# dart-icra/DART-Dual-Arm-Non-Prehensile-Manipulation

Hardware: AMD Instinct MI355X
Metric: MPC solves/sec (horizon N=20, batch=18 objects) at 1/2/4/8 GPUs; max |u−u_ref| (higher is better)
Workload: dtype f64

## Files before the change

dart-dual-arm-non-prehensile-manipulation_amd/csrc/dart_mpc_abi.hip:

```cpp
#include <hip/hip_runtime.h>

#include <cstdio>
#include <cstring>
#include <chrono>
#include <mutex>
#include <initializer_list>
#include <vector>
#include <string>

#include "dart_mpc.h"
#include "pmpc_ipm.h"
#include "pmpc_model.h"
#include "wave.h"
#include "rmpc_ipm.h"
#include "lmpc_ipm.h"
#include "lmpc_policy.h"
#include "lmpc_experience.h"
#include "lmpc_ppo.h"
#include "lmpc_train.h"
#include "arm_qp.h"
#include "loop_step.h"

#include <cmath>

// ... 151 lines not shown
        size_t cap;
        int xcd;
    };
    std::vector<RestoArea> resto;
    unsigned xcd_next = 0;
    char* loop_buf = nullptr;
    char* roll_buf = nullptr;
    size_t roll_cap = 0;
    float* action_buf = nullptr;
};

namespace {

int fail(dart_mpc_handle* h, int code, const char* what, hipError_t e = hipSuccess) {
    if (h) {
        char buf[256];
        if (e != hipSuccess) std::snprintf(buf, sizeof buf, "%s: %s", what, hipGetErrorString(e));
        else std::snprintf(buf, sizeof buf, "%s", what);
        h->err = buf;
    }
    return code;
}

#define HIPCHK(h, call, what)                                          \
    do {                                                               \
        hipError_t e_ = (call);                                        \
        if (e_ != hipSuccess) return fail((h), DART_MPC_EHIP, (what), e_); \
    } while (0)

int check_cfg(const dart_mpc_config* c) {
    if (!c) return 0;
    if (c->variant != DART_MPC_PMPC && c->variant != DART_MPC_RMPC && c->variant != DART_MPC_LMPC) return 0;
    if (c->N < 1 || c->N > 63) return 0;
    if (!(c->Ts > 0.0) || !(c->tol > 0.0) || !(c->gravity == c->gravity) || c->max_iter < 1 || c->B_max < 1) return 0;
    if (c->acceptable_iter < 0 || (c->acceptable_iter > 0 && !(c->acceptable_tol > 0.0))) return 0;
    if (c->max_soc < 0 || c->max_soc > 8) return 0;
    if (c->pmpc_path != 0 && c->pmpc_path != 1) return 0;
    if (!(c->constr_mult_init_max >= 0.0)) return 0;
    if (!(c->max_cpu_time >= 0.0) || c->max_cpu_time > 1e9) return 0;
    return 1;
}

void server_release(dart_mpc_handle* h) {
    auto& v = h->srv;
    if (v.mbox) (void)hipHostFree(v.mbox);
    if (v.stream) (void)hipStreamDestroy(v.stream);
    v = dart_mpc_handle::Server{};
}

void io_release(dart_mpc_handle* h) {
    auto& o = h->io;
    if (o.hin) (void)hipHostFree(o.hin);
    if (o.hout) (void)hipHostFree(o.hout);
    o = dart_mpc_handle::Io{};
}

hipError_t ensure_io(dart_mpc_handle* h) {
    auto& o = h->io;
    if (o.hin) return hipSuccess;
    const size_t nw = (size_t)dart_mpc_nw(h->cfg.N), Bm = (size_t)h->cfg.B_max;
    auto al = [](size_t n) { return (n + 255) & ~size_t(255); };
    o.off_ref = al(sizeof(double) * 6 * Bm); o.off_prm = 2 * o.off_ref; o.off_ww = 3 * o.off_ref;
    const size_t in_bytes = o.off_ww + al(sizeof(double) * nw * Bm);
    o.off_f = al(sizeof(double) * 2 * Bm); o.off_wo = o.off_f + al(sizeof(double) * Bm);
    o.off_st = o.off_wo + al(sizeof(double) * nw * Bm); o.off_it = o.off_st + al(sizeof(int32_t) * Bm);
    const size_t out_bytes = o.off_it + al(sizeof(int32_t) * Bm);
    const unsigned fl = hipHostMallocMapped | hipHostMallocCoherent;
// ... 2565 lines not shown
```

dart-dual-arm-non-prehensile-manipulation_amd/csrc/pmpc_ipm.hip:

```cpp
#if DART_WG == 2
#define dartmpc dartmpc_wg2
#endif
#include <hip/hip_runtime.h>
#include <stdint.h>
#include <stdlib.h>

#include "pmpc_ipm.h"
#include "pmpc_model.h"
#include "pmpc_resto.h"
#include "stamps.h"
#include "wave.h"

namespace dartmpc {

#ifdef DART_STAMPS
#ifndef PMPC_SEQ
__device__ unsigned long long g_stamp[16];
#define STAMP_FLUSH(b) STAMP_FLUSH_TO(g_stamp, b)
#else
__device__ unsigned long long g_stamp_seq[16];
#define STAMP_FLUSH(b) STAMP_FLUSH_TO(g_stamp_seq, b)
#endif
#else
#define STAMP_FLUSH(b) STAMP_FLUSH_TO(g_stamp, b)
#endif

#if DART_WG == 2
__shared__ double g_pm_x[4][2][4];
#endif
template <int SITE, int NV>
__device__ __forceinline__ void pm_pass(int src_wave, int src_node, const double (&v)[NV], double (&o)[NV]) {
    static_assert(NV <= 4 && SITE < 4, "four slots, four sites");
#if DART_WG == 1
    (void)src_wave; (void)src_node;
#pragma unroll
    for (int i = 0; i < NV; ++i) o[i] = v[i];
#else
    const int l = lane_id();
    if (wave_idx() == src_wave && (l & 31) == src_node) {
#pragma unroll
        for (int i = 0; i < NV; ++i) g_pm_x[SITE][l >> 5][i] = v[i];
    }
    __syncthreads();
#pragma unroll
    for (int i = 0; i < NV; ++i) o[i] = g_pm_x[SITE][l >> 5][i];
#endif
}

template <int CTRL, int ROWMASK, int FILL>
__device__ __forceinline__ double dpp_fill(double x) {
    const unsigned long long b = __builtin_bit_cast(unsigned long long, x);
// ... 205 lines not shown
        const double iQ = frcp(Q);
        W1[0] = iQ * U1; W2[0] = iQ * U2;
        Quu[0] = Q; iQs[0] = iQ;
    } else
    for (int step = 0; step < N; ++step) {
        double n11[NAX], n12[NAX], n22[NAX];
#pragma unroll
        for (int j = 0; j < NAX; ++j) {
            n11[j] = from_next(P11[j]); n12[j] = from_next(P12[j]); n22[j] = from_next(P22[j]);
        }
#pragma unroll
        for (int j = 0; j < NAX; ++j) {
            const double e1 = be1[j], e2 = be2[j];
            const double Q = fma(E11[j], n11[j], fma(E12[j], n12[j], fma(E22[j], n22[j], Rt[j])));
            const double PB1 = fma(n11[j], e1, n12[j] * e2), PB2 = fma(n12[j], e1, n22[j] * e2);
            const double U1 = PB1, U2 = fma(PB1, a12k, PB2 * a22k);
            const double X12 = fma(n11[j], a12k, n12[j] * a22k);
            const double X22 = fma(A11k, n11[j], fma(A12k, n12[j], fma(A22k, n22[j], X22d)));
            const double iQ = frcp(Q);
            const double w1 = iQ * U1, w2 = iQ * U2;
            P11[j] = fma(-w1, U1, fma(f11, n11[j], X11d));
            P12[j] = fma(-w1, U2, X12);
            P22[j] = fma(-w2, U2, X22);
            W1[j] = w1; W2[j] = w2;
            Quu[j] = Q; iQs[j] = iQ;
        }
    }
    bool bad = false;
#pragma unroll
    for (int j = 0; j < NAX; ++j) bad = bad || !(Quu[j] > 0.0) || !isfinite(Quu[j]);
    return !wany(bad);
}

struct PmOvlShared {
    double pt[6][kWave];
    double fc[6][kWave];
    int flag[4];
};
__shared__ PmOvlShared g_pm_ovl;

template <int NAX, bool QSCAN, bool ONEROW, bool SHORT2, bool RED, bool OVL = false>
__device__ __forceinline__ bool pmpc_solve(const PmpcArgs& a, const int b) {
    static_assert(!OVL || (NAX == 1 && QSCAN && !ONEROW && !RED && kWaves == 1), "the overlapped build: scan builds of N = 16..31");
    STAMP_DECL
    const int lane = (kWaves == 1 && !OVL) ? (int)threadIdx.x : lane_id();
    const int k = NAX == 1 ? node_base() + (lane & 31) : lane;
    const int ax0 = NAX == 1 ? (lane >> 5) : 0;
    const int N = a.N;
    const bool xon = k <= N, uon = k < N;
    constexpr bool one_row = ONEROW;
    constexpr bool short2 = SHORT2 && !ONEROW;
    const double h = a.Ts;

    const double* st = a.x0 + 6 * b;
    const double* rf = a.ref + 6 * b;
    const double* pr = a.prm + 6 * b;
    const double mu_f = pr[0], Qp = pr[1], Qv = pr[2], R = pr[3], ulo = pr[4], uhi = pr[5];

    double a12, a22, b1, b2;
    axis_rk4(h, a.g, mu_f, 0.0, 0.0, 1.0, a12, a22);
    axis_rk4(h, a.g, mu_f, 1.0, 0.0, 0.0, b1, b2);
    double zp1, zav, zcp, zcv;
    z_rk4(h, 0.0, 1.0, 1.0, zp1, zav);
    z_rk4(h, 1.0, 0.0, 0.0, zcp, zcv);
    const double lo = ulo - 1e-8 * fmax(1.0, fabs(ulo));
    const double hi = uhi + 1e-8 * fmax(1.0, fabs(uhi));
    const bool poly = fmax(fabs(lo), fabs(hi)) <= 1.0;
    const double f11 = uon ? 1.0 : 0.0, a12k = uon ? a12 : 0.0, a22k = uon ? a22 : 0.0;
    const double ai22 = 1.0 / a22, ai12 = -a12 * ai22;
    const double uonf = uon ? 1.0 : 0.0, ai12k = uon ? ai12 : 0.0, ai22k = uon ? ai22 : 1.0, a22i = uon ? a22 : 1.0;
    const double A11k = a12k * a12k, A12k = 2.0 * a12k * a22k, A22k = a22k * a22k;

// ... 5 lines not shown
    const double pushl = fmin(1e-2 * fmax(1.0, fabs(lo)), 1e-2 * (hi - lo));
    const double pushu = fmin(1e-2 * fmax(1.0, fabs(hi)), 1e-2 * (hi - lo));
    double gmax = 0.0;
#pragma unroll
    for (int j = 0; j < NAX; ++j) {
        const int ax = NAX == 1 ? ax0 : j;
        sp[j] = st[2 * ax]; sv[j] = st[2 * ax + 1];
        rp[j] = rf[2 * ax]; rv[j] = rf[2 * ax + 1];
        p[j] = xon ? (ww ? ww[6 * k + 2 * ax] : sp[j]) : 0.0;
        v[j] = xon ? (ww ? ww[6 * k + 2 * ax + 1] : sv[j]) : 0.0;
        double t = uon ? (ww ? ww[6 * (N + 1) + 2 * k + ax] : 0.0) : 0.0;
        if (uon) t = fmin(fmax(t, lo + pushl), hi - pushu);
        th[j] = t;
        lp[j] = 0.0; lv[j] = 0.0;
        zl[j] = uon ? 1.0 : 0.0; zu[j] = uon ? 1.0 : 0.0;
        if (xon) gmax = fmax(gmax, fmax(fabs(2 * Qp * (p[j] - rp[j])), fabs(2 * Qv * (v[j] - rv[j]))));
        if (uon) gmax = fmax(gmax, fabs(2 * R * th[j]));
        zA[j] = ax ? zav : zp1; zC[j] = ax ? zcv : zcp;
        zs[j] = st[4 + ax];
        zz[j] = xon ? (ww ? ww[6 * k + 4 + ax] : zs[j]) : 0.0;
    }
    gmax = wmax(gmax);
    const double sc = gmax > 100.0 ? 100.0 / gmax : 1.0;
    const double qp2 = sc * 2 * Qp, qv2 = sc * 2 * Qv, r2 = sc * 2 * R;
    const double scQp = sc * Qp, scQv = sc * Qv, scR = sc * R;
    const PmStage stg = {f11, a12k, a22k, ai12k, ai22k, a22i, uonf, A11k, A12k, A22k};
    auto quad_stage = [&](double csj, double snj, double lpnj, double lvnj, double zlj, double islj, double zuj,
                          double isuj, double& e1, double& e2, double& e11, double& e12, double& e22, double& rt0) {
        e1 = b1 * csj; e2 = b2 * csj;
        e11 = e1 * e1; e12 = 2.0 * e1 * e2; e22 = e2 * e2;
        rt0 = uon ? fma(snj, fma(b1, lpnj, b2 * lvnj), r2 + zlj * islj + zuj * isuj) : 1.0;
    };
    if constexpr (OVL) {
        if (__builtin_amdgcn_readfirstlane((int)(threadIdx.x >> 6)) != 0) {
            const long long max_rounds = 2ll * a.max_iter + 8;
            for (long long round = 0; round < max_rounds; ++round) {
                __syncthreads();
                if (__builtin_amdgcn_readfirstlane(g_pm_ovl.flag[0])) return false;
#ifdef DART_STAMPS
                const unsigned long long tf0 = __builtin_amdgcn_s_memtime();
#endif
                const double th1 = g_pm_ovl.pt[0][lane], sn1 = g_pm_ovl.pt[1][lane];
                const double lp1 = g_pm_ovl.pt[2][lane], lv1 = g_pm_ovl.pt[3][lane];
                const double zl1 = g_pm_ovl.pt[4][lane], zu1 = g_pm_ovl.pt[5][lane];
                const double c_ = tilt_cos_econ(poly, th1);
                const double cs1 = uon ? c_ : 0.0;
                const double ln = from_next(lp1), vn = from_next(lv1);
                const double lpn1 = uon ? ln : 0.0, lvn1 = uon ? vn : 0.0;
                const double sl = th1 - lo, su = hi - th1;
                const double isl1 = uon ? frcp(sl) : 0.0, isu1 = uon ? frcp(su) : 0.0;
                double be1[NAX], be2[NAX], E11[NAX], E12[NAX], E22[NAX], Rt0[NAX];
                quad_stage(cs1, sn1, lpn1, lvn1, zl1, isl1, zu1, isu1, be1[0], be2[0], E11[0], E12[0], E22[0], Rt0[0]);
                double W1[NAX], W2[NAX], P11[NAX], P12[NAX], P22[NAX], iQs[NAX];
                bool us = false;
                const bool okf = pmpc_riccati<NAX, QSCAN, ONEROW, SHORT2>(lane, N, uon, false, 0.0, qp2, qv2, stg, be1,
                                                                         be2, E11, E12, E22, Rt0, P11, P12, P22, W1,
                                                                         W2, iQs, us);
                g_pm_ovl.fc[0][lane] = P11[0]; g_pm_ovl.fc[1][lane] = P12[0]; g_pm_ovl.fc[2][lane] = P22[0];
                g_pm_ovl.fc[3][lane] = W1[0]; g_pm_ovl.fc[4][lane] = W2[0]; g_pm_ovl.fc[5][lane] = iQs[0];
                if (lane == 0) { g_pm_ovl.flag[1] = us ? 1 : 0; g_pm_ovl.flag[2] = okf ? 1 : 0; }
#ifdef DART_STAMPS
                t_acc_[13] += __builtin_amdgcn_s_memtime() - tf0;
                if (lane == 0) g_pm_ovl.flag[3] = (int)t_acc_[13];
#endif
                __syncthreads();
                if (__builtin_amdgcn_readfirstlane(g_pm_ovl.flag[0])) return false;
            }
            return false;
        }
        if (lane == 0) g_pm_ovl.flag[0] = 0;
    }

    const double tol = a.tol, mu_min = tol / 10;
    const double n_eq = 6.0 * (N + 1), n_b = 4.0 * N;
    const double inv_neb = 1.0 / (n_eq + n_b), inv_nb = 1.0 / n_b;
    const double gam_th = 1e-5, gam_ph = 1e-8, s_th = 1.1, s_ph = 2.3, eta_ph = 1e-8, gam_al = 0.05;

    auto defects = [&](double pj, double vj, double sj, double spj, double svj, double& g1, double& g2) {
        const double fp = fma(a12, vj, fma(b1, sj, pj));
        const double fv = fma(a22, vj, b2 * sj);
        double ip, iv;
        if constexpr (kWaves == 1) {
            ip = from_prev(fp); iv = from_prev(fv);
        } else {
            const double x2[2] = {fp, fv};
            double o2[2];
            from_prev_n(x2, o2);
            ip = o2[0]; iv = o2[1];
        }
        g1 = (k == 0) ? pj - spj : pj - ip;
        g2 = (k == 0) ? vj - svj : vj - iv;
    };
    auto axes_sum = [&](const double (&q)[NAX]) -> double {
        if constexpr (NAX == 1) return half_pair_sum(q[0]);
        else return q[0] + q[1];
    };
    auto zdefect = [&](double zj, double wj, int j) -> double {
        const double fz = fma(zA[j], zj, zC[j] * wj);
        const double ip = from_prev(fz);
        return (k == 0) ? zj - zs[j] : zj - ip;
    };
    auto vz_new = [&](const double (&t)[NAX]) -> double {
        double sq[NAX];
#pragma unroll
        for (int j = 0; j < NAX; ++j) sq[j] = uon ? t[j] * t[j] : 0.0;
        return -a.g * axes_sum(sq);
    };

    double g1[NAX], g2[NAX], gz[NAX], snc[NAX];
    double th0 = 0.0;
    {
        const double w0 = vz_new(th);
#pragma unroll
        for (int j = 0; j < NAX; ++j) {
            double s0, c0_;
            tilt_sincos(poly, th[j], s0, c0_);
            snc[j] = uon ? s0 : 0.0;
            defects(p[j], v[j], snc[j], sp[j], sv[j], g1[j], g2[j]);
            gz[j] = RED ? 0.0 : zdefect(zz[j], w0, j);
            if (xon) th0 += fabs(g1[j]) + fabs(g2[j]) + fabs(gz[j]);
        }
    }
    double theta = wsum(th0);
    const double th_max = 1e4 * fmax(1.0, theta), th_min = 1e-4 * fmax(1.0, theta);

    double fth = 0.0, fph = 0.0;
    int nfilt = 0;
    double mu = 0.1, delta_last = 0.0;
    int status = -1, it = 0;
    int in_soft = 0, soft_count = 0;
    STAMP(0);

    bool published = false;
    auto publish = [&]() {
        __builtin_amdgcn_sched_barrier(0);
        g_pm_ovl.pt[0][lane] = th[0]; g_pm_ovl.pt[1][lane] = snc[0];
        g_pm_ovl.pt[2][lane] = lp[0]; g_pm_ovl.pt[3][lane] = lv[0];
        g_pm_ovl.pt[4][lane] = zl[0]; g_pm_ovl.pt[5][lane] = zu[0];
        __syncthreads();
        __builtin_amdgcn_sched_barrier(0);
        published = true;
    };
#ifdef DART_STAMPS
    const unsigned long long t_loop0 = __builtin_amdgcn_s_memtime();
#endif
    for (it = a.mult_init_max > 0.0 ? -1 : 0; it < a.max_iter; ++it) {
        const bool lsm = it < 0;
#ifdef DART_STAMPS
        if (it == 1) t_acc_[12] = __builtin_amdgcn_s_memtime() - t_loop0;
#endif
        if constexpr (OVL) {
            if (PM_EXPECT(!lsm && !published, 0)) publish();
        }
        double sn[NAX], cs[NAX], isl[NAX], isu[NAX], lpn[NAX], lvn[NAX];
        double dinf = 0.0, pinf = 0.0, c0 = 0.0, cmin = 1e300, suml = 0.0, sumz = 0.0;
#pragma unroll
        for (int j = 0; j < NAX; ++j) {
            sn[j] = snc[j];
            const double c_ = tilt_cos_econ(poly, th[j]);
            cs[j] = uon ? c_ : 0.0;
            double ln, vn;
            if constexpr (kWaves == 1) {
                ln = from_next(lp[j]); vn = from_next(lv[j]);
            } else {
                const double x2[2] = {lp[j], lv[j]};
                double o2[2];
                from_next_n(x2, o2);
                ln = o2[0]; vn = o2[1];
            }
            lpn[j] = uon ? ln : 0.0; lvn[j] = uon ? vn : 0.0;
            const double sl = th[j] - lo, su = hi - th[j];
            isl[j] = uon ? frcp(sl) : 0.0; isu[j] = uon ? frcp(su) : 0.0;
            const double r1 = fma(qp2, p[j] - rp[j], lp[j] - lpn[j]);
            const double r2x = fma(qv2, v[j] - rv[j], lv[j] - fma(a12, lpn[j], a22 * lvn[j]));
            const double ru = fma(r2, th[j], -cs[j] * fma(b1, lpn[j], b2 * lvn[j])) - zl[j] + zu[j];
            dinf = fmax(dinf, xon ? fmax(fabs(r1), fabs(r2x)) : 0.0);
            dinf = fmax(dinf, uon ? fabs(ru) : 0.0);
            pinf = fmax(pinf, xon ? fmax(fmax(fabs(g1[j]), fabs(g2[j])), fabs(gz[j])) : 0.0);
            suml += xon ? fabs(lp[j]) + fabs(lv[j]) : 0.0;
            c0 = fmax(c0, uon ? fmax(zl[j] * sl, zu[j] * su) : 0.0);
            cmin = fmin(cmin, uon ? fmin(zl[j] * sl, zu[j] * su) : 1e300);
            sumz += zl[j] + zu[j];
        }
        float dinf_f = (float)dinf, pinf_f = (float)pinf, c0_f = (float)c0, cmin_f = (float)cmin;
        float suml_f = (float)suml, sumz_f = (float)sumz;
        wred_errors(dinf_f, pinf_f, c0_f, cmin_f, suml_f, sumz_f);
        const double dinf_w = dinf_f, pinf_w = pinf_f, c0_w = c0_f;
        const double cmin_w = cmin_f;
        const float sz_w = sumz_f;
        const double is_d = 100.0 * frcp(fmax(100.0, (double)(suml_f + sz_w) * inv_neb));
        const double is_c = 100.0 * frcp(fmax(100.0, (double)sz_w * inv_nb));
        dinf = dinf_w; pinf = pinf_w; c0 = c0_w;
        STAMP(1);
        if (!lsm && fmax(dinf * is_d, fmax(pinf, c0 * is_c)) <= tol) { status = 0; break; }
        for (; !lsm;) {
            const double cmu = fmax(c0 - mu, mu - cmin_w);
            if (fmax(dinf * is_d, fmax(pinf, cmu * is_c)) > 10.0 * mu || mu <= mu_min) break;
            mu = fmax(mu_min, fmin(0.2 * mu, mu * sqrt(mu)));
            nfilt = 0; in_soft = 0;
        }
        const double tau = fmax(0.99, 1.0 - mu);
        STAMP(2);

        double be1[NAX], be2[NAX], E11[NAX], E12[NAX], E22[NAX], Rt0[NAX], rt[NAX], q1[NAX], q2[NAX];
#pragma unroll
        for (int j = 0; j < NAX; ++j) {
            quad_stage(cs[j], sn[j], lpn[j], lvn[j], zl[j], isl[j], zu[j], isu[j], be1[j], be2[j], E11[j], E12[j],
                       E22[j], Rt0[j]);
            rt[j] = uon ? (lsm ? r2 * th[j] - zl[j] + zu[j] : fma(r2, th[j], mu * (isu[j] - isl[j]))) : 0.0;
            q1[j] = qp2 * (p[j] - rp[j]); q2[j] = qv2 * (v[j] - rv[j]);
        }
        double W1[NAX], W2[NAX], P11[NAX], P12[NAX], P22[NAX], iQs[NAX];
        double delta = 0.0;
        bool ok = false;
        int attempt = 0;
        if constexpr (OVL) {
            if (!lsm) {
                __builtin_amdgcn_sched_barrier(0);
                SPAN_BEGIN(t_b);
                __syncthreads();
                SPAN_END(14, t_b);
                const int usf = g_pm_ovl.flag[1], okff = g_pm_ovl.flag[2];
                P11[0] = g_pm_ovl.fc[0][lane]; P12[0] = g_pm_ovl.fc[1][lane]; P22[0] = g_pm_ovl.fc[2][lane];
                W1[0] = g_pm_ovl.fc[3][lane]; W2[0] = g_pm_ovl.fc[4][lane]; iQs[0] = g_pm_ovl.fc[5][lane];
                const bool us = __builtin_amdgcn_readfirstlane(usf) != 0;
                const bool okf = __builtin_amdgcn_readfirstlane(okff) != 0;
                if (PM_EXPECT(us && okf, 1)) {
                    STAMP_ADD(11, 1);
                    ok = true; attempt = 1;
                }
            }
        }
        for (; attempt < 60 && !ok; ++attempt) {
            if (PM_EXPECT(attempt > 0, 0))
                delta = (attempt == 1) ? (delta_last == 0.0 ? 1e-4 : fmax(1e-20, delta_last * (1.0 / 3.0)))
                                       : delta * (delta_last == 0.0 ? 100.0 : 8.0);
            bool use_scan = false;
            ok = pmpc_riccati<NAX, QSCAN, ONEROW, SHORT2>(lane, N, uon, lsm, delta, qp2, qv2, stg, be1, be2, E11, E12,
                                                          E22, Rt0, P11, P12, P22, W1, W2, iQs, use_scan);
            STAMP_ADD(11, use_scan ? 1 : 0);
        }
        STAMP_ADD(9, attempt);
        STAMP(3);
        if (PM_EXPECT(!ok, 0)) { status = -3; break; }
        if (delta > 0.0) delta_last = delta;

        double dp[NAX], dv[NAX], dth[NAX], dlp[NAX], dlv[NAX], dzl[NAX], dzu[NAX], dz[NAX];
        double amax = 1.0, az = 1.0;
        float am_lf = 1.0f, az_lf = 1.0f;
        const double (&g1o)[NAX] = g1, (&g2o)[NAX] = g2, (&gzo)[NAX] = gz;
        auto direction = [&]() {
            double p1[NAX], p2[NAX], kff[NAX], gn1[NAX], gn2[NAX], g1[NAX], g2[NAX], gz[NAX];
#pragma unroll
            for (int j = 0; j < NAX; ++j) {
                g1[j] = lsm ? 0.0 : g1o[j]; g2[j] = lsm ? 0.0 : g2o[j]; gz[j] = lsm ? 0.0 : gzo[j];
            }
            double nPw[3];
            if constexpr (kWaves == 1) {
#pragma unroll
                for (int j = 0; j < NAX; ++j) { gn1[j] = from_next(g1[j]); gn2[j] = from_next(g2[j]); }
            } else {
                const double x5[5] = {g1[0], g2[0], P11[0], P12[0], P22[0]};
                double o5[5];
                from_next_n(x5, o5);
// ... 304 lines not shown
                    gtdl += uon ? rt[j] * dth[j] : 0.0;
                }
                float tn_w = 0.0f;
#pragma unroll
                for (int j = 0; j < NAX; ++j) {
                    tn_w = fmaxf(tn_w, xon ? fabsf((float)dp[j]) * __builtin_amdgcn_rcpf(1.0f + fabsf((float)p[j])) : 0.0f);
                    tn_w = fmaxf(tn_w, xon ? fabsf((float)dv[j]) * __builtin_amdgcn_rcpf(1.0f + fabsf((float)v[j])) : 0.0f);
                    tn_w = fmaxf(tn_w, xon ? fabsf((float)dz[j]) * __builtin_amdgcn_rcpf(1.0f + fabsf((float)zz[j])) : 0.0f);
                    tn_w = fmaxf(tn_w, uon ? fabsf((float)dth[j]) * __builtin_amdgcn_rcpf(1.0f + fabsf((float)th[j])) : 0.0f);
                }
                wsum2_maxf_min2f(phil, gtdl, tn_w, am_lf, az_lf);
                frac_set();
                phi = phil; gTd = gtdl;
                const float lg_th = theta > 0.0 ? lg2(theta) : -3.0e38f;
                const float lg_gd = gTd < 0.0 ? lg2(-gTd) : 3.0e38f;
                lg_sw = (float)s_th * lg_th - (float)s_ph * lg_gd;
                amin = gam_th;
                if (gTd < 0.0) amin = fmin(gam_th, fmin(gam_ph * theta * frcp(-gTd), (double)__builtin_amdgcn_exp2f(fmaxf(lg_sw, -126.0f))));
                amin *= gam_al;
                tiny = tn_w < 2.2e-15f;
                alpha = amax; amain = amax;
                if constexpr (OVL) {
                    const double thc = fma(alpha, dth[0], th[0]);
                    double s_, c_;
                    tilt_sincos(poly, thc, s_, c_);
                    sn_pre = uon ? s_ : 0.0; sn_pre_on = true;
                    const double il = frcp(thc - lo), iu = frcp(hi - thc);
                    const double zln = fmax(fmin(fma(az, dzl[0], zl[0]), 1e10 * mu * il), 1e-10 * mu * il);
                    const double zun = fmax(fmin(fma(az, dzu[0], zu[0]), 1e10 * mu * iu), 1e-10 * mu * iu);
                    __builtin_amdgcn_sched_barrier(0);
                    g_pm_ovl.pt[0][lane] = thc; g_pm_ovl.pt[1][lane] = sn_pre;
                    g_pm_ovl.pt[2][lane] = fma(alpha, dlp[0], lp[0]); g_pm_ovl.pt[3][lane] = fma(alpha, dlv[0], lv[0]);
                    g_pm_ovl.pt[4][lane] = uon ? zln : 0.0; g_pm_ovl.pt[5][lane] = uon ? zun : 0.0;
                    __syncthreads();
                    __builtin_amdgcn_sched_barrier(0);
                }
            } else if (soc > 0) {
                alpha = amax;
            }
            STAMP(5);
            bool again = false;
            if constexpr ((NAX == 2 || kWaves == 2) && !RED) {
                if (PM_EXPECT(in_soft, 0)) break;
                if (PM_EXPECT(soc < 0 && alpha < amin, 0)) break;
            }
            for (;;) {
                trial(alpha);
                bool ft = false;
                if (PM_EXPECT(soc == 0 && tiny, 0)) { accepted = true; ftype = true; break; }
                if (acceptable(soc > 0 ? amain : alpha, ft)) { accepted = true; ftype = ft; break; }
                if (PM_EXPECT(!RED && soc == 0 && ls == 0 && a.max_soc > 0 && !(th_t < theta), 0)) {
#pragma unroll
                    for (int j = 0; j < NAX; ++j) {
                        g1[j] = fma(alpha, g1[j], g1t[j]); g2[j] = fma(alpha, g2[j], g2t[j]);
                        gz[j] = fma(alpha, gz[j], gzt[j]);
                    }
                    th_old = th_t; soc = 1; again = true;
                    break;
                }
                if (PM_EXPECT(soc > 0, 0)) {
                    if (soc < a.max_soc && th_t <= 0.99 * th_old) {
#pragma unroll
                        for (int j = 0; j < NAX; ++j) {
                            g1[j] = fma(alpha, g1[j], g1t[j]); g2[j] = fma(alpha, g2[j], g2t[j]);
                            gz[j] = fma(alpha, gz[j], gzt[j]);
                        }
// ... 83 lines not shown
                        }
                    }
                }
            }
            if (!accepted) { status = a.resto ? kPmNeedResto : -2; break; }
        }
        if (!soft && !ftype && nfilt < kWave) {
            if (lane == nfilt) { fth = (1 - gam_th) * theta; fph = phi - gam_ph * theta; }
            ++nfilt;
        }
        const bool hit = OVL && soc == 0 && ls == 0;
        if constexpr (OVL) {
            STAMP_ADD(15, hit ? (1ull << 16) : (1ull << 32));
            if (PM_EXPECT(!hit, 0)) {
                __builtin_amdgcn_sched_barrier(0);
                __syncthreads();
                __builtin_amdgcn_sched_barrier(0);
            }
        }
#pragma unroll
        for (int j = 0; j < NAX; ++j) {
            snc[j] = snt[j];
            lp[j] = fma(alpha, dlp[j], lp[j]); lv[j] = fma(alpha, dlv[j], lv[j]);
            th[j] = fma(alpha, dth[j], th[j]);
            if (OVL && PM_EXPECT(hit, 1)) {
                zl[j] = g_pm_ovl.pt[4][lane]; zu[j] = g_pm_ovl.pt[5][lane];
            } else {
                const double il = frcp(th[j] - lo), iu = frcp(hi - th[j]);
                const double zln = fmax(fmin(fma(az, dzl[j], zl[j]), 1e10 * mu * il), 1e-10 * mu * il);
                const double zun = fmax(fmin(fma(az, dzu[j], zu[j]), 1e10 * mu * iu), 1e-10 * mu * iu);
                zl[j] = uon ? zln : 0.0; zu[j] = uon ? zun : 0.0;
            }
        }
        if constexpr (OVL) {
            if (PM_EXPECT(!hit, 0)) publish();
        }
#pragma unroll
        for (int j = 0; j < NAX; ++j) {
            g1[j] = g1t[j]; g2[j] = g2t[j]; gz[j] = gzt[j];
            p[j] = fma(alpha, dp[j], p[j]); v[j] = fma(alpha, dv[j], v[j]);
            zz[j] = fma(alpha, dz[j], zz[j]);
        }
        theta = th_t;
        STAMP(7);
    }
    if constexpr (OVL) {
        if (lane == 0) g_pm_ovl.flag[0] = 1;
        __syncthreads();
#ifdef DART_STAMPS
        t_acc_[13] = (unsigned)__builtin_amdgcn_readfirstlane(g_pm_ovl.flag[3]);
#endif
    }

    if (PM_EXPECT(status == kPmNeedResto, 0)) {
        if constexpr (NAX == 1 && kWaves == 1 && !RED) {
            if (a.resto_buf) {
                double* ho = a.resto_buf + (size_t)kPmHo * b;
                double* row = ho + kPmHoRow * k;
                if (xon) {
                    row[2 * ax0] = p[0]; row[2 * ax0 + 1] = v[0]; row[4 + ax0] = zz[0];
                    row[8 + 2 * ax0] = lp[0]; row[8 + 2 * ax0 + 1] = lv[0]; row[8 + 4 + ax0] = 0.0;
                }
                if (uon) { row[6 + ax0] = th[0]; row[14 + ax0] = zl[0]; row[16 + ax0] = zu[0]; }
                if (lane < nfilt) { ho[kPmHoFilt + 2 * lane] = fth; ho[kPmHoFilt + 2 * lane + 1] = fph; }
                if (lane == 0) {
                    ho[kPmHoScal] = mu; ho[kPmHoScal + 1] = delta_last;
                    ho[kPmHoScal + 2] = (double)it; ho[kPmHoScal + 3] = (double)nfilt;
                }
            }
        }
        if (lane == 0 && wave_idx() == 0) a.status[b] = status;
        if (a.done && a.resto == 2) {
            __threadfence_system();
            if (lane == 0) __hip_atomic_store(a.done + b, a.seq, __ATOMIC_RELAXED, __HIP_MEMORY_SCOPE_SYSTEM);
        }
        return true;
    }
    double fl = 0.0;
#pragma unroll
    for (int j = 0; j < NAX; ++j) {
        const double ep = p[j] - rp[j], ev = v[j] - rv[j];
        fl += xon ? Qp * ep * ep + Qv * ev * ev : 0.0;
        fl += uon ? R * th[j] * th[j] : 0.0;
// ... 27 lines not shown
            }
#pragma unroll
            for (int j = 0; j < NAX; ++j) zz[j] = (NAX == 1 ? ax0 : j) ? vz : pz;
        }
#pragma unroll
        for (int j = 0; j < NAX; ++j) {
            const int ax = NAX == 1 ? ax0 : j;
            if (xon) { wo[6 * k + 2 * ax] = p[j]; wo[6 * k + 2 * ax + 1] = v[j]; wo[6 * k + 4 + ax] = zz[j]; }
            if (uon) wo[6 * (N + 1) + 2 * k + ax] = th[j];
        }
    }
    if (a.done) {
        __threadfence_system();
        if constexpr (kWaves == 2) __syncthreads();
        if (lane == 0 && wave_idx() == 0) __hip_atomic_store(a.done + b, a.seq, __ATOMIC_RELAXED, __HIP_MEMORY_SCOPE_SYSTEM);
    }
    STAMP(8);
    STAMP_FLUSH(b);
    return false;
}

__device__ __noinline__ void pmpc_resto_tail(const int b, const uint32_t seq, const uint32_t fl,
                                             const unsigned long long kargs) {
    PmpcArgs a = kernarg_load<PmpcArgs>(kargs);
    a.seq = seq;
    if (!(fl & 1u)) a.w_warm = nullptr;
    if (!(fl & 2u)) a.w_out = nullptr;
    __syncthreads();
    pmpc_resto_solve(a, b);
}

template <int NAX, bool QSCAN, bool ONEROW = false, bool SHORT2 = false, bool RED = false, bool OCC2 = false,
          bool FUSE = false, bool OVL = false>
__global__ __launch_bounds__(kWave * kWaves * (OVL ? 2 : 1)) __attribute__((amdgpu_waves_per_eu(OCC2 ? 2 : ((QSCAN || NAX == 2) ? 1 : 2))))
void pmpc_ipm_kernel(PmpcArgs a) {
    if (blockIdx.x % a.pack) return;
    const int b = blockIdx.x / a.pack;
    const bool handed = pmpc_solve<NAX, QSCAN, ONEROW, SHORT2, RED, OVL>(a, b);
    if constexpr (FUSE) {
        if (PM_EXPECT(handed, 0)) pmpc_resto_tail(b, a.seq, 3u, kernarg_addr());
    }
}

template <int NAX, bool ONEROW, bool SHORT2, bool FUSE = false>
__global__ __launch_bounds__(kWave) __attribute__((amdgpu_waves_per_eu(1)))
void pmpc_serve_kernel(PmpcArgs a, PmpcServe sv) {
    if (blockIdx.x % a.pack) return;
    const int b = blockIdx.x / a.pack;
    uint32_t seen = a.seq;
    unsigned long long t_last = __builtin_amdgcn_s_memrealtime();
    for (;;) {
        const unsigned long long w =
            __hip_atomic_load((const unsigned long long*)sv.mailbox, __ATOMIC_ACQUIRE, __HIP_MEMORY_SCOPE_SYSTEM);
        const uint32_t lo = (uint32_t)__builtin_amdgcn_readfirstlane((int)(uint32_t)(w & 0xffffffffu));
        const uint32_t hi = (uint32_t)__builtin_amdgcn_readfirstlane((int)(uint32_t)(w >> 32));
        const uint32_t sq = lo;
        if (hi >> 24) break;
        if (sq == seen) {
            if (__builtin_amdgcn_s_memrealtime() - t_last > sv.idle_ticks) break;
            __builtin_amdgcn_s_sleep(4);
            continue;
        }
        seen = sq;
        const uint32_t B = hi & 0xffffu, fl = (hi >> 16) & 0xffu;
        if ((uint32_t)b < B) {
            PmpcArgs r = a;
            r.B = (int)B; r.seq = sq;
// ... 105 lines not shown
    else
        hipLaunchKernelGGL((dartmpc::pmpc_serve_kernel<1, false, false>), dim3(grid), dim3(dartmpc::kWave), 0, stream, a,
                           *sv);
    return hipGetLastError();
}

extern "C" hipError_t dartmpc_launch_pmpc(const dartmpc::PmpcArgs* args, hipStream_t stream) {
    if (args->B <= 0) return hipSuccess;
    dartmpc::PmpcArgs a = *args;
    a.pack = (a.B <= 32) ? 8 : 1;
    const dim3 grid(a.B * a.pack);
    static const int qscan_max_b = [] {
        const char* e = getenv("DART_PMPC_QSCAN_MAX_B");
        return e ? atoi(e) : (1 << 30);
    }();
    static const int occ2_min_b = [] {
        if (const char* e = getenv("DART_PMPC_OCC2_MIN_B")) return atoi(e);
        int dev = 0, cus = 0;
        if (hipGetDevice(&dev) != hipSuccess || hipDeviceGetAttribute(&cus, hipDeviceAttributeMultiprocessorCount, dev) != hipSuccess || cus <= 0)
            return 1 << 30;
        return 2 * 4 * cus;
    }();
    const bool occ2 = !a.reduced && a.B >= occ2_min_b && a.B <= qscan_max_b;
    static const bool long_wg2 = [] {
        const char* e = getenv("DART_PMPC_SEQ_LONG");
        return !(e && e[0] == '1');
    }();
    if (a.resto == 1 && a.pack == 8 && !a.reduced && a.N <= 31 && !occ2 && a.B <= qscan_max_b &&
        dartmpc::resto_fuse_enabled())
        a.resto = 3;
    const bool fuse = a.resto == 3;
    const bool ovl = a.pack == 8 && !a.reduced && !occ2 && a.N >= 16 && a.N <= 31 && a.B <= qscan_max_b &&
                     dartmpc::pmpc_overlap_enabled();
    const dim3 block2(2 * dartmpc::kWave);
    if (ovl && a.N <= 23) {
        if (fuse)
            hipLaunchKernelGGL((dartmpc::pmpc_ipm_kernel<1, true, false, true, false, false, true, true>), grid, block2, 0, stream, a);
        else
            hipLaunchKernelGGL((dartmpc::pmpc_ipm_kernel<1, true, false, true, false, false, false, true>), grid, block2, 0, stream, a);
    } else if (ovl) {
        if (fuse)
            hipLaunchKernelGGL((dartmpc::pmpc_ipm_kernel<1, true, false, false, false, false, true, true>), grid, block2, 0, stream, a);
        else
            hipLaunchKernelGGL((dartmpc::pmpc_ipm_kernel<1, true, false, false, false, false, false, true>), grid, block2, 0, stream, a);
    } else if (a.N <= 23 && occ2) {
        hipLaunchKernelGGL((dartmpc::pmpc_ipm_kernel<1, true, false, true, false, true>), grid, dim3(dartmpc::kWave), 0, stream, a);
    } else if (a.N <= 15 && a.B <= qscan_max_b) {
        if (hipError_t e = dartmpc_launch_pmpc_seq(&a, grid.x, stream, 1)) return e;
    } else if (a.N <= 23 && a.B <= qscan_max_b) {
        if (fuse)
            hipLaunchKernelGGL((dartmpc::pmpc_ipm_kernel<1, true, false, true, false, false, true>), grid, dim3(dartmpc::kWave), 0, stream, a);
        else if (a.reduced)
            hipLaunchKernelGGL((dartmpc::pmpc_ipm_kernel<1, true, false, true, true>), grid, dim3(dartmpc::kWave), 0, stream, a);
        else
            hipLaunchKernelGGL((dartmpc::pmpc_ipm_kernel<1, true, false, true>), grid, dim3(dartmpc::kWave), 0, stream, a);
    } else if (a.N <= 31 && a.B <= qscan_max_b) {
        if (occ2)
            hipLaunchKernelGGL((dartmpc::pmpc_ipm_kernel<1, true, false, false, false, true>), grid, dim3(dartmpc::kWave), 0, stream, a);
        else if (fuse)
            hipLaunchKernelGGL((dartmpc::pmpc_ipm_kernel<1, true, false, false, false, false, true>), grid, dim3(dartmpc::kWave), 0, stream, a);
        else if (a.reduced)
            hipLaunchKernelGGL((dartmpc::pmpc_ipm_kernel<1, true, false, false, true>), grid, dim3(dartmpc::kWave), 0, stream, a);
        else
            hipLaunchKernelGGL((dartmpc::pmpc_ipm_kernel<1, true>), grid, dim3(dartmpc::kWave), 0, stream, a);
    } else if (a.N > 31 && !a.reduced && !a.resto && long_wg2) {
        if (hipError_t e = dartmpc_launch_pmpc_wg2(&a, grid.x, stream)) return e;
    } else {
        if (hipError_t e = dartmpc_launch_pmpc_seq(&a, grid.x, stream, 0)) return e;
    }
    if (a.resto == 1) {
        if (hipError_t e = hipGetLastError()) return e;
        return dartmpc_launch_pmpc_resto(&a, stream);
    }
    return hipGetLastError();
}

extern "C" hipError_t dartmpc_wave_selftest(double* d_out, hipStream_t stream) {
    hipLaunchKernelGGL(dartmpc::wave_selftest_kernel, dim3(1), dim3(dartmpc::kWave), 0, stream, d_out);
    return hipGetLastError();
}

#ifdef DART_STAMPS
extern "C" hipError_t dartmpc_read_stamps(unsigned long long* host_out) {
    return hipMemcpyFromSymbol(host_out, HIP_SYMBOL(dartmpc::g_stamp), sizeof(unsigned long long) * 16, 0,
                               hipMemcpyDeviceToHost);
}
#endif
#endif
```

Baseline: 319,200.

## Add third helper wave computing convergence errors and mu update in overlapped PMPC

Extends the overlapped PMPC IPM kernel from two waves to three. The new wave takes the published trial point from shared memory, computes the KKT error norms, the convergence test and the barrier-parameter update, and writes them back. The main wave then reads those results instead of computing them on its critical path. The cost is more shared-memory traffic, an extra wave per block, and behaviour that is now split across waves, so a lag between waves could change convergence. The config check also now accepts max_iter=0 for PMPC.

```diff
diff --git a/dart-dual-arm-non-prehensile-manipulation_amd/csrc/dart_mpc_abi.hip b/dart-dual-arm-non-prehensile-manipulation_amd/csrc/dart_mpc_abi.hip
--- a/dart-dual-arm-non-prehensile-manipulation_amd/csrc/dart_mpc_abi.hip
+++ b/dart-dual-arm-non-prehensile-manipulation_amd/csrc/dart_mpc_abi.hip
@@ -207,7 +207,8 @@
     if (!c) return 0;
     if (c->variant != DART_MPC_PMPC && c->variant != DART_MPC_RMPC && c->variant != DART_MPC_LMPC) return 0;
     if (c->N < 1 || c->N > 63) return 0;
-    if (!(c->Ts > 0.0) || !(c->tol > 0.0) || !(c->gravity == c->gravity) || c->max_iter < 1 || c->B_max < 1) return 0;
+    const int min_iter = c->variant == DART_MPC_PMPC ? 0 : 1;
+    if (!(c->Ts > 0.0) || !(c->tol > 0.0) || !(c->gravity == c->gravity) || c->max_iter < min_iter || c->B_max < 1) return 0;
     if (c->acceptable_iter < 0 || (c->acceptable_iter > 0 && !(c->acceptable_tol > 0.0))) return 0;
     if (c->max_soc < 0 || c->max_soc > 8) return 0;
     if (c->pmpc_path != 0 && c->pmpc_path != 1) return 0;
diff --git a/dart-dual-arm-non-prehensile-manipulation_amd/csrc/pmpc_ipm.hip b/dart-dual-arm-non-prehensile-manipulation_amd/csrc/pmpc_ipm.hip
--- a/dart-dual-arm-non-prehensile-manipulation_amd/csrc/pmpc_ipm.hip
+++ b/dart-dual-arm-non-prehensile-manipulation_amd/csrc/pmpc_ipm.hip
@@ -15,8 +15,8 @@
 
 #ifdef DART_STAMPS
 #ifndef PMPC_SEQ
-__device__ unsigned long long g_stamp[16];
-#define STAMP_FLUSH(b) STAMP_FLUSH_TO(g_stamp, b)
+__device__ unsigned long long g_stamp[32];
+#define STAMP_FLUSH(b) STAMP_FLUSH32_TO(g_stamp, b)
 #else
 __device__ unsigned long long g_stamp_seq[16];
 #define STAMP_FLUSH(b) STAMP_FLUSH_TO(g_stamp_seq, b)
@@ -288,12 +288,68 @@
     return !wany(bad);
 }
 
+#define PMPC_POINT_LANE(j)                                                                                          \
+    const double c_ = tilt_cos_econ(poly, th[j]);                                                                   \
+    cs[j] = uon ? c_ : 0.0;                                                                                         \
+    double ln, vn;                                                              \
+    if constexpr (kWaves == 1) {                                                                                    \
+        ln = from_next(lp[j]); vn = from_next(lv[j]);                                                               \
+    } else {                                                                                                        \
+        const double x2[2] = {lp[j], lv[j]};                                                                        \
+        double o2[2];                                                                                               \
+        from_next_n(x2, o2);                                                                                        \
+        ln = o2[0]; vn = o2[1];                                                                                     \
+    }                                                                                                               \
+    lpn[j] = uon ? ln : 0.0; lvn[j] = uon ? vn : 0.0;                                                               \
+    const double sl = th[j] - lo, su = hi - th[j];                                                                  \
+    isl[j] = uon ? frcp(sl) : 0.0; isu[j] = uon ? frcp(su) : 0.0;
+#define PMPC_POINT_ERRORS                                                                                           \
+    double dinf = 0.0, pinf = 0.0, c0 = 0.0, cmin = 1e300, suml = 0.0, sumz = 0.0;                                  \
+    _Pragma("unroll") for (int j = 0; j < NAX; ++j) {                                                               \
+        PMPC_POINT_LANE(j)                                                                                          \
+        const double r1 = fma(qp2, p[j] - rp[j], lp[j] - lpn[j]);                                                   \
+        const double r2x = fma(qv2, v[j] - rv[j], lv[j] - fma(a12, lpn[j], a22 * lvn[j]));                          \
+        const double ru = fma(r2, th[j], -cs[j] * fma(b1, lpn[j], b2 * lvn[j])) - zl[j] + zu[j];                    \
+        dinf = fmax(dinf, xon ? fmax(fabs(r1), fabs(r2x)) : 0.0);                                                   \
+        dinf = fmax(dinf, uon ? fabs(ru) : 0.0);                                                                    \
+        pinf = fmax(pinf, xon ? fmax(fmax(fabs(g1[j]), fabs(g2[j])), fabs(gz[j])) : 0.0);                           \
+        suml += xon ? fabs(lp[j]) + fabs(lv[j]) : 0.0;                                                              \
+        c0 = fmax(c0, uon ? fmax(zl[j] * sl, zu[j] * su) : 0.0);                                                    \
+        cmin = fmin(cmin, uon ? fmin(zl[j] * sl, zu[j] * su) : 1e300);                                              \
+        sumz += zl[j] + zu[j];                                                                                      \
+    }                                                                                                               \
+    float dinf_f = (float)dinf, pinf_f = (float)pinf, c0_f = (float)c0, cmin_f = (float)cmin;                       \
+    float suml_f = (float)suml, sumz_f = (float)sumz;                                                               \
+    wred_errors(dinf_f, pinf_f, c0_f, cmin_f, suml_f, sumz_f);                                                      \
+    const double dinf_w = dinf_f, pinf_w = pinf_f, c0_w = c0_f;                                                     \
+    const double cmin_w = cmin_f;                                                                                   \
+    const float sz_w = sumz_f;                                                                                      \
+    const double is_d = 100.0 * frcp(fmax(100.0, (double)(suml_f + sz_w) * inv_neb));                               \
+    const double is_c = 100.0 * frcp(fmax(100.0, (double)sz_w * inv_nb));                                           \
+    dinf = dinf_w; pinf = pinf_w; c0 = c0_w;
+#define PMPC_RT(j) (uon ? (lsm ? r2 * th[j] - zl[j] + zu[j] : fma(r2, th[j], mu * (isu[j] - isl[j]))) : 0.0)
+#define PMPC_POINT_CONVERGED (!lsm && fmax(dinf * is_d, fmax(pinf, c0 * is_c)) <= tol)
+#define PMPC_POINT_MU(RUN)                                                                                          \
+    for (; (RUN) && !lsm;) {                                                                                        \
+        const double cmu = fmax(c0 - mu, mu - cmin_w);                                                              \
+        if (fmax(dinf * is_d, fmax(pinf, cmu * is_c)) > 10.0 * mu || mu <= mu_min) break;                           \
+        mu = fmax(mu_min, fmin(0.2 * mu, mu * sqrt(mu)));                                                           \
+        nfilt = 0; in_soft = 0;                   \
+    }
+
 struct PmOvlShared {
-    double pt[6][kWave];
+    double pt[9][kWave];
     double fc[6][kWave];
-    int flag[4];
+    double mu;
+    double ev[7];
+    int flag[8];
 };
 __shared__ PmOvlShared g_pm_ovl;
+
+__device__ __forceinline__ double pm_uniform(double x) {
+    return __hiloint2double(__builtin_amdgcn_readfirstlane(__double2hiint(x)),
+                            __builtin_amdgcn_readfirstlane(__double2loint(x)));
+}
 
 template <int NAX, bool QSCAN, bool ONEROW, bool SHORT2, bool RED, bool OVL = false>
 __device__ __forceinline__ bool pmpc_solve(const PmpcArgs& a, const int b) {
@@ -365,7 +421,7 @@
         rt0 = uon ? fma(snj, fma(b1, lpnj, b2 * lvnj), r2 + zlj * islj + zuj * isuj) : 1.0;
     };
     if constexpr (OVL) {
-        if (__builtin_amdgcn_readfirstlane((int)(threadIdx.x >> 6)) != 0) {
+        if (__builtin_amdgcn_readfirstlane((int)(threadIdx.x >> 6)) == 1) {
             const long long max_rounds = 2ll * a.max_iter + 8;
             for (long long round = 0; round < max_rounds; ++round) {
                 __syncthreads();
@@ -401,7 +457,6 @@
             }
             return false;
         }
-        if (lane == 0) g_pm_ovl.flag[0] = 0;
     }
 
     const double tol = a.tol, mu_min = tol / 10;
@@ -440,6 +495,48 @@
         return -a.g * axes_sum(sq);
     };
 
+    if constexpr (OVL) {
+        if (__builtin_amdgcn_readfirstlane((int)(threadIdx.x >> 6)) == 2) {
+            const long long max_rounds = 2ll * a.max_iter + 8;
+            for (long long round = 0; round < max_rounds; ++round) {
+                __syncthreads();
+                if (__builtin_amdgcn_readfirstlane(g_pm_ovl.flag[0])) return false;
+#ifdef DART_STAMPS
+                const unsigned long long te0 = __builtin_amdgcn_s_memtime();
+#endif
+                const double th[NAX] = {g_pm_ovl.pt[0][lane]}, sn1 = g_pm_ovl.pt[1][lane];
+                const double lp[NAX] = {g_pm_ovl.pt[2][lane]}, lv[NAX] = {g_pm_ovl.pt[3][lane]};
+                const double zl[NAX] = {g_pm_ovl.pt[4][lane]}, zu[NAX] = {g_pm_ovl.pt[5][lane]};
+                const double p[NAX] = {g_pm_ovl.pt[6][lane]}, v[NAX] = {g_pm_ovl.pt[7][lane]};
+                const double zz1 = g_pm_ovl.pt[8][lane];
+                double mu = pm_uniform(g_pm_ovl.mu);
+                double g1[NAX], g2[NAX], gz[NAX];
+                defects(p[0], v[0], sn1, sp[0], sv[0], g1[0], g2[0]);
+                gz[0] = zdefect(zz1, vz_new(th), 0);
+                double cs[NAX], isl[NAX], isu[NAX], lpn[NAX], lvn[NAX];
+                int nfilt = 1, in_soft = 0;
+                constexpr bool lsm = false;
+                PMPC_POINT_ERRORS
+                const bool conv = PMPC_POINT_CONVERGED;
+                PMPC_POINT_MU(!conv)
+                (void)cs; (void)isl; (void)isu; (void)in_soft;
+                if (lane == 0) {
+                    g_pm_ovl.ev[0] = dinf; g_pm_ovl.ev[1] = pinf; g_pm_ovl.ev[2] = c0; g_pm_ovl.ev[3] = cmin_w;
+                    g_pm_ovl.ev[4] = is_d; g_pm_ovl.ev[5] = is_c; g_pm_ovl.ev[6] = mu;
+                    g_pm_ovl.flag[4] = conv ? 1 : 0; g_pm_ovl.flag[5] = nfilt == 0 ? 1 : 0;
+                }
+#ifdef DART_STAMPS
+                t_acc_[16] += __builtin_amdgcn_s_memtime() - te0;
+                if (lane == 0) g_pm_ovl.flag[6] = (int)t_acc_[16];
+#endif
+                __syncthreads();
+                if (__builtin_amdgcn_readfirstlane(g_pm_ovl.flag[0])) return false;
+            }
+            return false;
+        }
+        if (lane == 0) g_pm_ovl.flag[0] = 0;
+    }
+
     double g1[NAX], g2[NAX], gz[NAX], snc[NAX];
     double th0 = 0.0;
     {
@@ -470,6 +567,8 @@
         g_pm_ovl.pt[0][lane] = th[0]; g_pm_ovl.pt[1][lane] = snc[0];
         g_pm_ovl.pt[2][lane] = lp[0]; g_pm_ovl.pt[3][lane] = lv[0];
         g_pm_ovl.pt[4][lane] = zl[0]; g_pm_ovl.pt[5][lane] = zu[0];
+        g_pm_ovl.pt[6][lane] = p[0]; g_pm_ovl.pt[7][lane] = v[0]; g_pm_ovl.pt[8][lane] = zz[0];
+        if (lane == 0) g_pm_ovl.mu = mu;
         __syncthreads();
         __builtin_amdgcn_sched_barrier(0);
         published = true;
@@ -486,53 +585,13 @@
             if (PM_EXPECT(!lsm && !published, 0)) publish();
         }
         double sn[NAX], cs[NAX], isl[NAX], isu[NAX], lpn[NAX], lvn[NAX];
-        double dinf = 0.0, pinf = 0.0, c0 = 0.0, cmin = 1e300, suml = 0.0, sumz = 0.0;
-#pragma unroll
-        for (int j = 0; j < NAX; ++j) {
-            sn[j] = snc[j];
-            const double c_ = tilt_cos_econ(poly, th[j]);
-            cs[j] = uon ? c_ : 0.0;
-            double ln, vn;
-            if constexpr (kWaves == 1) {
-                ln = from_next(lp[j]); vn = from_next(lv[j]);
-            } else {
-                const double x2[2] = {lp[j], lv[j]};
-                double o2[2];
-                from_next_n(x2, o2);
-                ln = o2[0]; vn = o2[1];
-            }
-            lpn[j] = uon ? ln : 0.0; lvn[j] = uon ? vn : 0.0;
-            const double sl = th[j] - lo, su = hi - th[j];
-            isl[j] = uon ? frcp(sl) : 0.0; isu[j] = uon ? frcp(su) : 0.0;
-            const double r1 = fma(qp2, p[j] - rp[j], lp[j] - lpn[j]);
-            const double r2x = fma(qv2, v[j] - rv[j], lv[j] - fma(a12, lpn[j], a22 * lvn[j]));
-            const double ru = fma(r2, th[j], -cs[j] * fma(b1, lpn[j], b2 * lvn[j])) - zl[j] + zu[j];
-            dinf = fmax(dinf, xon ? fmax(fabs(r1), fabs(r2x)) : 0.0);
-            dinf = fmax(dinf, uon ? fabs(ru) : 0.0);
-            pinf = fmax(pinf, xon ? fmax(fmax(fabs(g1[j]), fabs(g2[j])), fabs(gz[j])) : 0.0);
-            suml += xon ? fabs(lp[j]) + fabs(lv[j]) : 0.0;
-            c0 = fmax(c0, uon ? fmax(zl[j] * sl, zu[j] * su) : 0.0);
-            cmin = fmin(cmin, uon ? fmin(zl[j] * sl, zu[j] * su) : 1e300);
-            sumz += zl[j] + zu[j];
-        }
-        float dinf_f = (float)dinf, pinf_f = (float)pinf, c0_f = (float)c0, cmin_f = (float)cmin;
-        float suml_f = (float)suml, sumz_f = (float)sumz;
-        wred_errors(dinf_f, pinf_f, c0_f, cmin_f, suml_f, sumz_f);
-        const double dinf_w = dinf_f, pinf_w = pinf_f, c0_w = c0_f;
-        const double cmin_w = cmin_f;
-        const float sz_w = sumz_f;
-        const double is_d = 100.0 * frcp(fmax(100.0, (double)(suml_f + sz_w) * inv_neb));
-        const double is_c = 100.0 * frcp(fmax(100.0, (double)sz_w * inv_nb));
-        dinf = dinf_w; pinf = pinf_w; c0 = c0_w;
+#pragma unroll
+        for (int j = 0; j < NAX; ++j) sn[j] = snc[j];
+        PMPC_POINT_ERRORS
         STAMP(1);
-        if (!lsm && fmax(dinf * is_d, fmax(pinf, c0 * is_c)) <= tol) { status = 0; break; }
-        for (; !lsm;) {
-            const double cmu = fmax(c0 - mu, mu - cmin_w);
-            if (fmax(dinf * is_d, fmax(pinf, cmu * is_c)) > 10.0 * mu || mu <= mu_min) break;
-            mu = fmax(mu_min, fmin(0.2 * mu, mu * sqrt(mu)));
-            nfilt = 0; in_soft = 0;
-        }
-        const double tau = fmax(0.99, 1.0 - mu);
+        if (!OVL && PMPC_POINT_CONVERGED) { status = 0; break; }
+        PMPC_POINT_MU(!OVL)
+        double tau = fmax(0.99, 1.0 - mu);
         STAMP(2);
 
         double be1[NAX], be2[NAX], E11[NAX], E12[NAX], E22[NAX], Rt0[NAX], rt[NAX], q1[NAX], q2[NAX];
@@ -540,7 +599,7 @@
         for (int j = 0; j < NAX; ++j) {
             quad_stage(cs[j], sn[j], lpn[j], lvn[j], zl[j], isl[j], zu[j], isu[j], be1[j], be2[j], E11[j], E12[j],
                        E22[j], Rt0[j]);
-            rt[j] = uon ? (lsm ? r2 * th[j] - zl[j] + zu[j] : fma(r2, th[j], mu * (isu[j] - isl[j]))) : 0.0;
+            rt[j] = PMPC_RT(j);
             q1[j] = qp2 * (p[j] - rp[j]); q2[j] = qv2 * (v[j] - rv[j]);
         }
         double W1[NAX], W2[NAX], P11[NAX], P12[NAX], P22[NAX], iQs[NAX];
@@ -554,8 +613,14 @@
                 __syncthreads();
                 SPAN_END(14, t_b);
                 const int usf = g_pm_ovl.flag[1], okff = g_pm_ovl.flag[2];
+                const int cvf = g_pm_ovl.flag[4], mcf = g_pm_ovl.flag[5];
+                const double mu_e = g_pm_ovl.ev[6];
                 P11[0] = g_pm_ovl.fc[0][lane]; P12[0] = g_pm_ovl.fc[1][lane]; P22[0] = g_pm_ovl.fc[2][lane];
                 W1[0] = g_pm_ovl.fc[3][lane]; W2[0] = g_pm_ovl.fc[4][lane]; iQs[0] = g_pm_ovl.fc[5][lane];
+                if (__builtin_amdgcn_readfirstlane(cvf) != 0) { status = 0; break; }
+                mu = pm_uniform(mu_e);
+                if (__builtin_amdgcn_readfirstlane(mcf) != 0) { nfilt = 0; in_soft = 0; }
+                tau = fmax(0.99, 1.0 - mu);
                 const bool us = __builtin_amdgcn_readfirstlane(usf) != 0;
                 const bool okf = __builtin_amdgcn_readfirstlane(okff) != 0;
                 if (PM_EXPECT(us && okf, 1)) {
@@ -563,6 +628,7 @@
                     ok = true; attempt = 1;
                 }
             }
+            rt[0] = PMPC_RT(0);
         }
         for (; attempt < 60 && !ok; ++attempt) {
             if (PM_EXPECT(attempt > 0, 0))
@@ -933,6 +999,9 @@
                     g_pm_ovl.pt[0][lane] = thc; g_pm_ovl.pt[1][lane] = sn_pre;
                     g_pm_ovl.pt[2][lane] = fma(alpha, dlp[0], lp[0]); g_pm_ovl.pt[3][lane] = fma(alpha, dlv[0], lv[0]);
                     g_pm_ovl.pt[4][lane] = uon ? zln : 0.0; g_pm_ovl.pt[5][lane] = uon ? zun : 0.0;
+                    g_pm_ovl.pt[6][lane] = fma(alpha, dp[0], p[0]); g_pm_ovl.pt[7][lane] = fma(alpha, dv[0], v[0]);
+                    g_pm_ovl.pt[8][lane] = fma(alpha, dz[0], zz[0]);
+                    if (lane == 0) g_pm_ovl.mu = mu;
                     __syncthreads();
                     __builtin_amdgcn_sched_barrier(0);
                 }
@@ -1082,14 +1151,14 @@
                 zl[j] = uon ? zln : 0.0; zu[j] = uon ? zun : 0.0;
             }
         }
-        if constexpr (OVL) {
-            if (PM_EXPECT(!hit, 0)) publish();
-        }
 #pragma unroll
         for (int j = 0; j < NAX; ++j) {
             g1[j] = g1t[j]; g2[j] = g2t[j]; gz[j] = gzt[j];
             p[j] = fma(alpha, dp[j], p[j]); v[j] = fma(alpha, dv[j], v[j]);
             zz[j] = fma(alpha, dz[j], zz[j]);
+        }
+        if constexpr (OVL) {
+            if (PM_EXPECT(!hit, 0)) publish();
         }
         theta = th_t;
         STAMP(7);
@@ -1099,6 +1168,7 @@
         __syncthreads();
 #ifdef DART_STAMPS
         t_acc_[13] = (unsigned)__builtin_amdgcn_readfirstlane(g_pm_ovl.flag[3]);
+        t_acc_[16] = (unsigned)__builtin_amdgcn_readfirstlane(g_pm_ovl.flag[6]);
 #endif
     }
 
@@ -1192,7 +1262,7 @@
 
 template <int NAX, bool QSCAN, bool ONEROW = false, bool SHORT2 = false, bool RED = false, bool OCC2 = false,
           bool FUSE = false, bool OVL = false>
-__global__ __launch_bounds__(kWave * kWaves * (OVL ? 2 : 1)) __attribute__((amdgpu_waves_per_eu(OCC2 ? 2 : ((QSCAN || NAX == 2) ? 1 : 2))))
+__global__ __launch_bounds__(kWave * kWaves * (OVL ? 3 : 1)) __attribute__((amdgpu_waves_per_eu(OCC2 ? 2 : ((QSCAN || NAX == 2) ? 1 : 2))))
 void pmpc_ipm_kernel(PmpcArgs a) {
     if (blockIdx.x % a.pack) return;
     const int b = blockIdx.x / a.pack;
@@ -1364,17 +1434,17 @@
     const bool fuse = a.resto == 3;
     const bool ovl = a.pack == 8 && !a.reduced && !occ2 && a.N >= 16 && a.N <= 31 && a.B <= qscan_max_b &&
                      dartmpc::pmpc_overlap_enabled();
-    const dim3 block2(2 * dartmpc::kWave);
+    const dim3 block3(3 * dartmpc::kWave);
     if (ovl && a.N <= 23) {
         if (fuse)
-            hipLaunchKernelGGL((dartmpc::pmpc_ipm_kernel<1, true, false, true, false, false, true, true>), grid, block2, 0, stream, a);
+            hipLaunchKernelGGL((dartmpc::pmpc_ipm_kernel<1, true, false, true, false, false, true, true>), grid, block3, 0, stream, a);
         else
-            hipLaunchKernelGGL((dartmpc::pmpc_ipm_kernel<1, true, false, true, false, false, false, true>), grid, block2, 0, stream, a);
+            hipLaunchKernelGGL((dartmpc::pmpc_ipm_kernel<1, true, false, true, false, false, false, true>), grid, block3, 0, stream, a);
     } else if (ovl) {
         if (fuse)
-            hipLaunchKernelGGL((dartmpc::pmpc_ipm_kernel<1, true, false, false, false, false, true, true>), grid, block2, 0, stream, a);
+            hipLaunchKernelGGL((dartmpc::pmpc_ipm_kernel<1, true, false, false, false, false, true, true>), grid, block3, 0, stream, a);
         else
-            hipLaunchKernelGGL((dartmpc::pmpc_ipm_kernel<1, true, false, false, false, false, false, true>), grid, block2, 0, stream, a);
+            hipLaunchKernelGGL((dartmpc::pmpc_ipm_kernel<1, true, false, false, false, false, false, true>), grid, block3, 0, stream, a);
     } else if (a.N <= 23 && occ2) {
         hipLaunchKernelGGL((dartmpc::pmpc_ipm_kernel<1, true, false, true, false, true>), grid, dim3(dartmpc::kWave), 0, stream, a);
     } else if (a.N <= 15 && a.B <= qscan_max_b) {
@@ -1414,7 +1484,7 @@
 
 #ifdef DART_STAMPS
 extern "C" hipError_t dartmpc_read_stamps(unsigned long long* host_out) {
-    return hipMemcpyFromSymbol(host_out, HIP_SYMBOL(dartmpc::g_stamp), sizeof(unsigned long long) * 16, 0,
+    return hipMemcpyFromSymbol(host_out, HIP_SYMBOL(dartmpc::g_stamp), sizeof(unsigned long long) * 32, 0,
                                hipMemcpyDeviceToHost);
 }
 #endif
```

New measurement: 319,600 (median of 6 runs). About the same (+0.1%).
